# adamchang2000/DenseFusion

Hardware: AMD Instinct MI355X
Metric: poses/sec (node) YCB-Video 1000 pts + 2 refine iters (higher is better)
Workload: dtype f32

## Files before the change

densefusion_amd/_lib.py:

```python
from __future__ import annotations

import ctypes
import os

_HERE = os.path.dirname(os.path.abspath(__file__))
LIB_PATH = os.path.join(_HERE, "libdfusion_hip_dev.so" if os.environ.get("DF_DEV_LIB") else "libdfusion_hip.so")
_lib = None

_vp, _i, _i64, _f, _sz = ctypes.c_void_p, ctypes.c_int, ctypes.c_int64, ctypes.c_float, ctypes.c_size_t

class ConvDesc(ctypes.Structure):
    _fields_ = ([(n, ctypes.c_void_p) for n in ("in_", "wgt", "bias", "res", "prelu", "out")] +
                [(n, ctypes.c_int32) for n in ("B", "H", "W", "Cin", "in_ld", "in_coff", "OH", "OW", "Cout", "out_ld",
                                               "out_coff", "res_ld", "res_coff", "KH", "KW", "stride", "pad", "dil",
                                               "act")] +
                [("splitk_ws", ctypes.c_void_p), ("splitk_ws_bytes", ctypes.c_size_t)])


SIGNATURES = {
    "df_last_error": (ctypes.c_char_p, []),
    "df_version": (_i, []),
    "df_knn_device": (_i, [_vp, _i, _vp, _i, _i, _i, _vp, _vp]),
    "df_knn": (_i, [_vp, _vp, _vp, _i, _i, _i, _i, _i, _vp]),
    "knn_device": (None, [_vp, _i, _vp, _i, _i, _i, _vp, _vp, _vp]),
# ... 73 lines not shown
    "df_conv_route": (_i, [ctypes.POINTER(ConvDesc), _i, _vp, _vp, _vp, _i, _i, _i, _i, _vp]),
    "df_conv3x3_winograd_scratch_bytes": (ctypes.c_size_t, [ctypes.POINTER(ConvDesc)]),
    "df_conv3x3_winograd_nhwc": (_i, [ctypes.POINTER(ConvDesc), _vp, ctypes.c_size_t, _vp]),
    "df_wino_route": (_i, [_i, _i, _i, _i, _i]),
    "df_wino_tiles": (ctypes.c_long, [_i, _i, _i, _i, _i, ctypes.POINTER(_i), ctypes.POINTER(_i)]),
    "df_wino_axis_map": (_i, [_i, _i, _i, _i]),
    "df_trainer_create": (_vp, [_i, _i, _i]),
    "df_trainer_destroy": (None, [_vp]),
    "df_trainer_flat_numel": (_i64, [_vp]),
    "df_trainer_num_params": (_i, [_vp]),
    "df_trainer_param_info": (_i, [_vp, _i, ctypes.c_char_p, _i, ctypes.POINTER(_i64), ctypes.POINTER(_i)]),
    "df_trainer_pack_param": (_i, [_vp, ctypes.c_char_p, _vp, _vp, _vp]),
    "df_trainer_unpack_param": (_i, [_vp, ctypes.c_char_p, _vp, _vp, _vp]),
    "df_posenet_train_workspace_bytes": (_sz, [_vp, _i, _i, _i, _i]),
    "df_posenet_train_step": (_i, [_vp, _vp, _vp, _i64, _i, _i, _i] + [_vp] * 6 + [_i, _vp, _f, _i, ctypes.c_uint] + [_vp] * 9 + [_sz, _vp]),
    "df_posenet_train_multi_workspace_bytes": (_sz, [_vp, _i, _vp, _vp, _vp, _i]),
    "df_posenet_train_step_multi": (_i, [_vp, _vp, _vp, _i64, _i, _vp, _vp, _vp, _vp] + [_vp] * 5 + [_i, _vp, _f, _i, ctypes.c_uint] + [_vp] * 9 + [_sz, _vp]),
    "df_trainer_set_splitk": (_i, [_vp, _i]),
    "df_trainer_profile": (_i, [_vp, _i]),
    "df_trainer_profile_read": (_i, [_vp, ctypes.POINTER(ctypes.c_double), ctypes.POINTER(ctypes.c_double), ctypes.POINTER(_i)]),
    "df_refiner_train_workspace_bytes": (_sz, [_vp, _i, _i]),
    "df_refiner_train_step": (_i, [_vp, _vp, _vp, _i64, _i] + [_vp] * 5 + [_i, _vp] + [_vp] * 4 + [_sz, _vp]),
    "df_conv3x3_winograd_tile_scratch_bytes": (ctypes.c_size_t, [ctypes.POINTER(ConvDesc), _i]),
    "df_conv3x3_winograd_tile_nhwc": (_i, [ctypes.POINTER(ConvDesc), _i, _vp, ctypes.c_size_t, _vp]),
    "df_conv2d_dgrad_nhwc": (_i, [ctypes.POINTER(ConvDesc), _vp, _vp, _vp, _i, _vp]),
    "df_conv2d_wgrad_workspace_bytes": (ctypes.c_size_t, [ctypes.POINTER(ConvDesc)]),
    "df_conv2d_wgrad_nhwc": (_i, [ctypes.POINTER(ConvDesc), _vp, _vp, _vp, _vp, ctypes.c_size_t, _vp]),
    "df_net_debug_taps": (_i, [_vp, _i]),
    "df_net_debug_tap_read": (_i, [_vp, ctypes.c_char_p, _vp, _i64, ctypes.POINTER(_i64)]),
    "df_net_profile": (_i, [_vp, _i]),
    "df_net_profile_read": (_i, [_vp] + [ctypes.POINTER(ctypes.c_double)] * 4 + [ctypes.POINTER(_i)]),
    "df_net_profile_read_split": (_i, [_vp] + [ctypes.POINTER(ctypes.c_double)] * 3 + [ctypes.POINTER(_i)]),
    "df_gemm_route": (_i, [_i, _i, _i]),
    "df_segment_scratch_bytes": (_sz, [_i, _i, _i, _i]),
    "df_segment_input": (_i, [_vp, _vp, _i, _i, _i, _vp]),
    "df_segment_detect": (_i, [_vp, _vp, _i, _i, _i, _i, _i, _i, _i, _vp, _vp, _vp, _vp, _vp, _sz, _vp]),
    "df_seg_batch_scratch_bytes": (_sz, [_i, _i, _i, _i]),
    "df_seg_batch": (_i, [_vp, _vp, _i, _i, _i, _vp, _i, _i, _i, _vp, _i, _i, _vp, _i, _i, _i, _i, _i, _vp, _vp, _vp, _vp, _sz, _vp]),
    "df_seg_score_block_pixels": (_i, []),
    "df_seg_score": (_i, [_vp, _vp, _i, _i, _i, _i, _i, _vp, _vp, _vp, _vp]),
    "df_seg_masks": (_i, [_vp, _i, _i, _i, _vp, _vp, _i, _i, _i, _vp, _vp]),
    "df_mesh_closest_tile_triangles": (_i, []),
    "df_mesh_closest_scratch_bytes": (_sz, [_i]),
    "df_mesh_closest": (_i, [_vp, _i, _vp, _i, _vp, _i, _vp, _i, _vp, _vp, _vp, _vp, _sz, _vp]),
    "df_fp64_rate_probe": (_i, [_i, _i, _vp, _vp]),
}


def lib():
    global _lib
    if _lib is None:
        if not os.path.exists(LIB_PATH):
            raise RuntimeError(
                f"{LIB_PATH} not found: the HIP extension is not built. Run "
                "`python -c 'import __graft_entry__ as g; g.build()'` at the repo root (needs hipcc). "
                "densefusion_amd has no CPU fallback.")
        L = ctypes.CDLL(LIB_PATH)
        for name, (res, args) in SIGNATURES.items():
            fn = getattr(L, name)
            fn.restype, fn.argtypes = res, args
        _lib = L
    return _lib


def check(status: int, what: str = "") -> None:
    if status != 0:
# ... 38 lines not shown
```

densefusion_amd/csrc/conv_api.hip:

```cpp
#include <vector>

#include "igemm.h"
#include "wino.h"

using namespace df;

extern "C" int df_gemm_route(int n, int k, int epilogue) { return split_route(n, k, epilogue); }

static void desc_fields(const df_conv_desc *d, ConvParams &p) {
  p.in = d->in; p.wgt = d->wgt; p.bias = d->bias; p.res = d->res; p.prelu = d->prelu; p.out = d->out;
  p.B = d->B; p.H = d->H; p.W = d->W; p.Cin = d->Cin; p.in_ld = d->in_ld; p.in_coff = d->in_coff;
  p.OH = d->OH; p.OW = d->OW; p.Cout = d->Cout; p.out_ld = d->out_ld; p.out_coff = d->out_coff;
  p.res_ld = d->res_ld; p.res_coff = d->res_coff;
  p.KH = d->KH; p.KW = d->KW; p.stride = d->stride; p.pad = d->pad; p.dil = d->dil; p.act = d->act;
}

static int conv_desc_to_params(const df_conv_desc *d, ConvParams &p, const char *what) {
  if (!d) return set_error(DF_ERR_ARG, "%s: null descriptor", what);
  if (d->KH != d->KW) return set_error(DF_ERR_ARG, "%s: square kernels only", what);
  desc_fields(d, p);
  if (p.OH != conv_out(p.H, p.KH, p.stride, p.pad, p.dil) || p.OW != conv_out(p.W, p.KW, p.stride, p.pad, p.dil))
    return set_error(DF_ERR_ARG, "%s: OH/OW do not match the convolution geometry", what);
  return DF_OK;
}

static thread_local int t_last_splitk = 1;
extern "C" int df_conv_last_splitk(void) { return t_last_splitk; }

extern "C" int df_conv2d_nhwc(const df_conv_desc *d, df_stream_t stream) {
  ConvParams p;
  int rc = conv_desc_to_params(d, p, "conv2d_nhwc");
  if (rc != DF_OK) return rc;
  if (p.act == ACT_PRELU && !p.prelu) return set_error(DF_ERR_ARG, "conv2d_nhwc: PReLU needs a slope");
  p.splitk_ws = static_cast<float *>(d->splitk_ws); p.splitk_ws_bytes = d->splitk_ws ? d->splitk_ws_bytes : 0;
  ConvRoute taken;
  rc = launch_conv(p, to_stream(stream), &taken);
  t_last_splitk = taken.splitk;
  return rc;
}

// ... 191 lines not shown
```

densefusion_amd/csrc/igemm.h:

```cpp
#pragma once
#include "common.h"

namespace df {

enum Act { ACT_NONE = 0, ACT_RELU = 1, ACT_PRELU = 2 };

struct ConvParams {
  const float *in = nullptr;
  const float *wgt = nullptr;
  const float *bias = nullptr;
  const float *res = nullptr;
  const float *prelu = nullptr;
  float *out = nullptr;
  float *colsum = nullptr;
  int B = 1, H = 1, W = 1, Cin = 0, in_ld = 0, in_coff = 0;
  int OH = 1, OW = 1, Cout = 0, out_ld = 0, out_coff = 0;
  int res_ld = 0, res_coff = 0;
  int KH = 1, KW = 1, stride = 1, pad = 0, dil = 1;
  int up = 1;
  int act = ACT_NONE;
  int rows_per_group = 0, rows_valid = 0, bias_group_ld = 0;
  int zcount = 1;
  long z_in_coff = 0, z_wgt = 0, z_bias = 0, z_out_coff = 0;
  const void *wpl = nullptr;
// ... 13 lines not shown
  q.B = f.B; q.H = f.OH; q.W = f.OW; q.Cin = f.Cout; q.OH = f.H; q.OW = f.W; q.Cout = f.Cin;
  q.KH = f.KH; q.KW = f.KW; q.stride = 1; q.up = f.stride; q.dil = f.dil; q.pad = f.dil * (f.KH - 1) - f.pad;
  return q;
}

struct WgradSeg { int B, H, W, OH, OW; long in_row0, out_row0; };

enum ConvKernel { CONV_NONE = 0, CONV_V1 = 1, CONV_V2 = 2, CONV_V4 = 3, CONV_V4_COLSUM = 4, CONV_V4_MULTI = 5, CONV_BF16 = 6 };
struct ConvRoute {
  int kernel = CONV_NONE;
  int bm = 0, bn = 0;
  int loader = 0;
  int splitk = 1;
  int wgroup = 0;
  int nseg = 1;
};
int conv_route(const ConvParams &p, int nseg, const WgradSeg *segs, int first, ConvRoute &r);
int launch_conv(const ConvParams &p, hipStream_t st, ConvRoute *taken = nullptr);

constexpr int CONV_MAX_BUCKETS = 16;
int launch_conv_multi(const ConvParams &p, int nseg, const WgradSeg *segs, hipStream_t st);

size_t wgrad_workspace_bytes(const ConvParams &p);
int launch_wgrad(const ConvParams &p, float *dw, float *db, void *ws, size_t ws_bytes, hipStream_t st, int accumulate = 0);

constexpr int WGRAD_MAX_SEGS = 32;
size_t wgrad_multi_workspace_bytes(const ConvParams &p, int nseg, const WgradSeg *segs);
int launch_wgrad_multi(const ConvParams &p, int nseg, const WgradSeg *segs, float *dw, float *db, void *ws, size_t ws_bytes, hipStream_t st,
                       int accumulate = 0);

enum GemmEpi { GEMM_EPI_PLAIN = 0, GEMM_EPI_RESIDUAL = 1, GEMM_EPI_GROUPS = 2, GEMM_EPI_OTHER = 3 };
int gemm_epi_kind(const ConvParams &p);
int split_route(int N, int K, int epi);
void cut_weight_planes(const float *w, void *planes, long elems, long stride, hipStream_t st);
int try_split_gemm(const ConvParams &p, hipStream_t st, ConvRoute &r);

}
```

densefusion_amd/csrc/split_gemm.hip:

```cpp
#include "igemm.h"
#include <atomic>
#include <cstdint>
#ifdef DF_DEV
#include <map>
#include <mutex>
#include <tuple>
#endif

namespace df {
namespace {

typedef __bf16 bf16x8 __attribute__((ext_vector_type(8)));
typedef __bf16 bf16x2 __attribute__((ext_vector_type(2)));
typedef float f32x16 __attribute__((ext_vector_type(16)));
typedef float f32x2 __attribute__((ext_vector_type(2)));

constexpr int SBM = 128, SBN = 128, SBK = 32;
constexpr int PLANE_BYTES = 128 * 64;

__device__ __forceinline__ void cut3(float a0, float a1, unsigned &hi, unsigned &mid, unsigned &lo) {
  const bf16x2 h = __builtin_convertvector(f32x2{a0, a1}, bf16x2);
  hi = __builtin_bit_cast(unsigned, h);
  const float r0 = a0 - __builtin_bit_cast(float, hi << 16), r1 = a1 - __builtin_bit_cast(float, hi & 0xFFFF0000u);
  const bf16x2 m = __builtin_convertvector(f32x2{r0, r1}, bf16x2);
// ... 7 lines not shown
__device__ __forceinline__ void cut4(const float4 &x, uint4 &h, uint4 &m, uint4 &l) {
  if (H == 0) { cut3(x.x, x.y, h.x, m.x, l.x); cut3(x.z, x.w, h.y, m.y, l.y); }
  else { cut3(x.x, x.y, h.z, m.z, l.z); cut3(x.z, x.w, h.w, m.w, l.w); }
}
__device__ __forceinline__ void cut8(const float4 &x0, const float4 &x1, uint4 &h, uint4 &m, uint4 &l) { cut4<0>(x0, h, m, l); cut4<1>(x1, h, m, l); }

__host__ __device__ constexpr int pair_a(int q) { constexpr int t[6] = {2, 0, 1, 1, 0, 0}; return t[q]; }
__host__ __device__ constexpr int pair_b(int q) { constexpr int t[6] = {0, 2, 1, 0, 1, 0}; return t[q]; }
__device__ __forceinline__ f32x16 mfma_pair(const bf16x8 (&fa)[3], const bf16x8 (&fb)[3], int q, f32x16 c) {
  return __builtin_amdgcn_mfma_f32_32x32x16_bf16(fa[pair_a(q)], fb[pair_b(q)], c, 0, 0, 0);
}
constexpr bool pair_brings_new_planes(int q) {
  for (int r = 0; r < q; ++r)
    if (pair_a(r) == pair_a(q) || pair_b(r) == pair_b(q)) return false;
  return true;
}
static_assert(pair_brings_new_planes(0) && pair_brings_new_planes(1) && pair_brings_new_planes(2), "pairs 0..2 must reach all planes of A and of B");

__global__ void cut_planes_kernel(const float *__restrict__ w, __bf16 *__restrict__ planes, long elems, long stride) {
  const long i = (long)blockIdx.x * blockDim.x + threadIdx.x;
  if (i >= elems) return;
  unsigned h, m, l;
  cut3(w[i], 0.f, h, m, l);
  unsigned short *pl = reinterpret_cast<unsigned short *>(planes);
  pl[i] = (unsigned short)h; pl[stride + i] = (unsigned short)m; pl[2 * stride + i] = (unsigned short)l;
}

struct SplitArgs {
  const float *in; const __bf16 *wpl; const float *bias; const float *res; const float *prelu; float *out; float *colsum;
  long M, wplane;
  int N, K, in_ld, in_coff, out_ld, out_coff, res_ld, res_coff, act, rows_per_group, rows_valid, bias_group_ld;
  long z_in_coff, z_wgt, z_bias, z_out_coff;
  int tiles_m, tiles_n;
  long cs_rows;
};

__device__ __forceinline__ int piece(int row, int slot) { return row * 64 + ((slot ^ ((row >> 2) & 3)) << 4); }

struct SplitTile { int tm, tn, z; const float *in; const __bf16 *wpl; };
__device__ __forceinline__ bool split_tile(const SplitArgs &a, SplitTile &t) {
  const int xcd = blockIdx.x & 7, seq = blockIdx.x >> 3;
  t.tm = (seq / a.tiles_n) * 8 + xcd;
  t.tn = seq % a.tiles_n;
  t.z = blockIdx.z;
  t.in = a.in + t.z * a.z_in_coff + a.in_coff;
  t.wpl = a.wpl + t.z * a.z_wgt;
  return t.tm < a.tiles_m;
}

#define SPLIT_FETCH3(p0, p1, p2, g, k0)                                          \
  do {                                                                           \
    p0 = *reinterpret_cast<const uint4 *>((g) + (k0));                           \
    p1 = *reinterpret_cast<const uint4 *>((g) + a.wplane + (k0));                \
    p2 = *reinterpret_cast<const uint4 *>((g) + 2 * a.wplane + (k0));            \
  } while (0)
#define SPLIT_STORE3(base, stride, off, p0, p1, p2)                              \
  do {                                                                           \
    *reinterpret_cast<uint4 *>((base) + (off)) = p0;                             \
    *reinterpret_cast<uint4 *>((base) + (stride) + (off)) = p1;                  \
    *reinterpret_cast<uint4 *>((base) + 2 * (stride) + (off)) = p2;              \
  } while (0)
#define SPLIT_FRAG_OFFSETS(b0)                                                   \
  int offa[2][2], offb[2][2];                                                    \
  _Pragma("unroll") for (int ks = 0; ks < 2; ++ks)                               \
  _Pragma("unroll") for (int t = 0; t < 2; ++t) {                                \
    offa[ks][t] = piece(wr * 64 + t * 32 + fr, ks * 2 + fh);                     \
    offb[ks][t] = (b0) + piece(wc * 64 + t * 32 + fr, ks * 2 + fh);              \
  }
#define SPLIT_READ_FRAGS(base, apl, bpl)                                                                  \
  bf16x8 fa[2][3], fb[2][3];                                                                              \
  _Pragma("unroll") for (int t = 0; t < 2; ++t)                                                           \
  _Pragma("unroll") for (int p = 0; p < 3; ++p) {                                                         \
    fa[t][p] = *reinterpret_cast<const bf16x8 *>((base) + p * (apl) + offa[ks][t]);                       \
    fb[t][p] = *reinterpret_cast<const bf16x8 *>((base) + p * (bpl) + offb[ks][t]);                       \
  }
#define SPLIT_STAGE_ROLES(half)                                                  \
  const int srow0 = tid >> 2, srow1 = srow0 + (half), sslot = tid & 3;           \
  const int soff0 = piece(srow0, sslot), soff1 = piece(srow1, sslot);            \
  long r0 = row0 + srow0, r1 = row0 + srow1;                                     \
  r0 = r0 < a.M ? r0 : a.M - 1;                                                  \
// ... 59 lines not shown
  const EpiRules ru = epi_rules(a, z, row0, wrow);
  float *out = a.out + z * a.z_out_coff + a.out_coff;
#pragma unroll
  for (int j = 0; j < 2; ++j) {
    const int n = nb + j * 32 + fr;
    const float b1 = ru.bias ? ru.bias[n] : 0.f;
    float csum = 0.f;
#pragma unroll
    for (int i = 0; i < 2; ++i) {
      const int tb = wrow + i * 32 + 4 * fh;
      const long mb = row0 + tb;
      float r[16];
      if (a.res) {
#pragma unroll
        for (int e = 0; e < 16; ++e) {
          long m = mb + (e & 3) + 8 * (e >> 2);
          m = m < a.M ? m : a.M - 1;
          r[e] = a.res[m * a.res_ld + a.res_coff + n];
        }
      }
#pragma unroll
      for (int e = 0; e < 16; ++e) {
        const int tr = tb + (e & 3) + 8 * (e >> 2);
        const long m = row0 + tr;
        const float v = epi_finish(acc[i][j][e], &b1, a.res ? &r[e] : nullptr, a.act, ru.slope);
        if (a.out && m < a.M) out[m * a.out_ld + n] = v;
        csum += tr < ru.limit ? v : 0.f;
      }
    }
    epi_colsum(a, ru, z, n, fh, csum);
  }
}

__device__ __forceinline__ void split_epilogue_rows(const SplitArgs &a, const f32x16 (&acc)[2][2], int z, long row0, int wrow, int nb, int lane, float *blk) {
  const int fr = lane & 31, fh = lane >> 5;
  const EpiRules ru = epi_rules(a, z, row0, wrow);
#pragma unroll
  for (int j = 0; j < 2; ++j) {
    const int n = nb + j * 32 + fr;
    const float b1 = ru.bias ? ru.bias[n] : 0.f;
    float csum = 0.f;
#pragma unroll
    for (int i = 0; i < 2; ++i)
#pragma unroll
      for (int e = 0; e < 16; ++e) {
        const int br = i * 32 + 4 * fh + (e & 3) + 8 * (e >> 2);
        const float v = a.res ? epi_finish(acc[i][j][e], &b1, nullptr, ACT_NONE, 0.f) : epi_finish(acc[i][j][e], &b1, nullptr, a.act, ru.slope);
        blk[br * 64 + j * 32 + fr] = v;
        csum += wrow + br < ru.limit ? v : 0.f;
      }
    epi_colsum(a, ru, z, n, fh, csum);
  }
  if (!a.out) return;
  __builtin_amdgcn_fence(__ATOMIC_RELEASE, "wavefront");
  __builtin_amdgcn_wave_barrier();
  __builtin_amdgcn_fence(__ATOMIC_ACQUIRE, "wavefront");
  float *out = a.out + z * a.z_out_coff + a.out_coff;
  const int c4 = (lane & 15) * 4;
#pragma unroll 4
  for (int it = 0; it < 16; ++it) {
    const int br = it * 4 + (lane >> 4);
    const long m = row0 + wrow + br;
    float4 v = *reinterpret_cast<const float4 *>(blk + br * 64 + c4);
    if (m < a.M) {
      if (a.res) {
        const float4 r = *reinterpret_cast<const float4 *>(a.res + m * a.res_ld + a.res_coff + nb + c4);
        epi_finish(reinterpret_cast<float (&)[4]>(v), nullptr, &r.x, a.act, ru.slope);
      }
      *reinterpret_cast<float4 *>(out + m * a.out_ld + nb + c4) = v;
    }
  }
  __builtin_amdgcn_fence(__ATOMIC_RELEASE, "wavefront");
  __builtin_amdgcn_wave_barrier();
}

__global__ __launch_bounds__(256, 2) void gemm_split_bf16_kernel(const SplitArgs a) {
  __shared__ __attribute__((aligned(16))) unsigned char lds[6 * PLANE_BYTES];
  const int tid = threadIdx.x, lane = tid & 63, wave = tid >> 6;
  SplitTile wg;
  if (!split_tile(a, wg)) return;
  const long row0 = (long)wg.tm * SBM;
  const int n0 = wg.tn * SBN;

  SPLIT_STAGE_ROLES(64);
  const __bf16 *bg1 = wg.wpl + (long)(n0 + srow1) * a.K + sslot * 8;
// ... 93 lines not shown
    __builtin_amdgcn_sched_group_barrier(0x020, 7, 0);                           \
    __builtin_amdgcn_sched_group_barrier(0x100, 12, 0);                          \
    _Pragma("unroll") for (int g = 0; g < 48; ++g) {                             \
      __builtin_amdgcn_sched_group_barrier(0x008, 1, 0);                         \
      __builtin_amdgcn_sched_group_barrier(0x002, 2, 0);                         \
      if (g >= 8 && g < 32 && (g & 1) == 0) __builtin_amdgcn_sched_group_barrier(0x100, 1, 0); \
      if (g % 5 == 4) __builtin_amdgcn_sched_group_barrier(0x200, 1, 0);         \
    }                                                                            \
    __syncthreads();                                                             \
  } while (0)

  unsigned char *const st0 = lds2, *const st1 = lds2 + V2_STAGE;
  const int nk = a.K / SBK;
  const int klast = a.K - SBK;
  V2_FETCH(x, 0);
  V2_FETCH(y, SBK < klast ? SBK : klast);
  V2_STAGE_TO(x, st0);
  __syncthreads();
  int kt = 0;
  for (; kt + 1 < nk; kt += 2) {
    const int k2 = (kt + 2) * SBK, k3 = (kt + 3) * SBK;
    V2_BODY(x, y, k2 < klast ? k2 : klast, st0, st1);
    V2_BODY(y, x, k3 < klast ? k3 : klast, st1, st0);
  }
  if (nk & 1) { V2_COMPUTE(st0); }
  split_epilogue(a, acc, wg.z, row0, wr * 64, n0 + wc * 64, fr, fh);
}

constexpr int V3_PL = 256 * 32, V3_STAGE = 6 * V3_PL;
constexpr int V3_LDS = 8 * 64 * 64 * 4;

__device__ __forceinline__ int piece16(int row, int half) { return row * 32 + ((half ^ ((row >> 3) & 1)) << 4); }

__global__ __launch_bounds__(512, 1) void gemm_split_bf16_v3_kernel(const SplitArgs a) {
  extern __shared__ __attribute__((aligned(16))) unsigned char lds3[];
  const int tid = threadIdx.x, lane = tid & 63, wave = tid >> 6;
  SplitTile wg;
  if (!split_tile(a, wg)) return;
  const long row0 = (long)wg.tm * 256;
  const int n0 = wg.tn * 256;

  const int srow = tid >> 1, shalf = tid & 1;
  const int soff = piece16(srow, shalf);
  long r = row0 + srow;
  r = r < a.M ? r : a.M - 1;
  const float *ag = wg.in + r * a.in_ld + shalf * 8;
  const __bf16 *bg = wg.wpl + (long)(n0 + srow) * a.K + shalf * 8;
  float4 xa0, xa1, ya0, ya1;
  uint4 b0, b1, b2;
#define V3_FETCH_A(S, k0)                                                        \
  do {                                                                           \
    S##a0 = *reinterpret_cast<const float4 *>(ag + (k0));                        \
    S##a1 = *reinterpret_cast<const float4 *>(ag + (k0) + 4);                    \
  } while (0)
#define V3_FETCH_B(k0) SPLIT_FETCH3(b0, b1, b2, bg, k0)
#define V3_PIN(v) asm volatile("" : "+v"(v.x), "+v"(v.y), "+v"(v.z), "+v"(v.w))
#define V3_CUT0(S) do { V3_PIN(S##a0); cut4<0>(S##a0, ch, cm, cl); } while (0)
#define V3_CUT1(S) do { V3_PIN(S##a1); cut4<1>(S##a1, ch, cm, cl); } while (0)
#define V3_WRITE_A(base) SPLIT_STORE3(base, V3_PL, soff, ch, cm, cl)
#define V3_WRITE_B(base) SPLIT_STORE3((base) + 3 * V3_PL, V3_PL, soff, b0, b1, b2)

  const int wr = wave >> 2, wc = wave & 3, fr = lane & 31, fh = lane >> 5;
  f32x16 acc[2][2][2] = {};
  const int offa = piece16(wr * 128 + fr, fh), offb = 3 * V3_PL + piece16(wc * 64 + fr, fh);
#define V3_READ(base, q)                                                                                  \
  do {                                                                                                    \
    _Pragma("unroll") for (int t = 0; t < 4; ++t)                                                         \
      fa[t][pair_a(q)] = *reinterpret_cast<const bf16x8 *>((base) + pair_a(q) * V3_PL + offa + t * 1024); \
    _Pragma("unroll") for (int t = 0; t < 2; ++t)                                                         \
      fb[t][pair_b(q)] = *reinterpret_cast<const bf16x8 *>((base) + pair_b(q) * V3_PL + offb + t * 1024); \
  } while (0)
#define V3_MFMA(q)                                                                                        \
  do {                                                                                                    \
    _Pragma("unroll") for (int i = 0; i < 4; ++i)                                                         \
    _Pragma("unroll") for (int j = 0; j < 2; ++j) acc[i >> 1][i & 1][j] = mfma_pair(fa[i], fb[j], q, acc[i >> 1][i & 1][j]); \
  } while (0)
#define V3_WEAVE(n, mask, cnt)                                                   \
  do {                                                                           \
    _Pragma("unroll") for (int g = 0; g < (n); ++g) {                            \
      __builtin_amdgcn_sched_group_barrier(0x008, 1, 0);                         \
      __builtin_amdgcn_sched_group_barrier(mask, cnt, 0);                        \
    }                                                                            \
    __builtin_amdgcn_sched_barrier(0);                                           \
  } while (0)
#define V3_BODY(FS, SS, ka, kb, cur, nxt)                                        \
  do {                                                                           \
    bf16x8 fa[4][3], fb[2][3];                                                   \
    uint4 ch, cm, cl;                                                            \
    V3_FETCH_B(kb);                                                              \
    V3_FETCH_A(FS, ka);                                                          \
    V3_READ(cur, 0);                                                             \
    __builtin_amdgcn_sched_barrier(0);                                           \
    V3_READ(cur, 1);                                                             \
    V3_MFMA(0);                                                                  \
    V3_WEAVE(6, 0x100, 1);                                                       \
    V3_READ(cur, 2);                                                             \
    V3_MFMA(1);                                                                  \
    V3_WEAVE(6, 0x100, 1);                                                       \
    V3_CUT0(SS);                                                                 \
    V3_MFMA(2);                                                                  \
    V3_WEAVE(8, 0x002, 3);                                                       \
    V3_CUT1(SS);                                                                 \
    V3_MFMA(3);                                                                  \
    V3_WEAVE(8, 0x002, 3);                                                       \
    V3_WRITE_A(nxt);                                                             \
    V3_MFMA(4);                                                                  \
    V3_WEAVE(3, 0x200, 1);                                                       \
    V3_WRITE_B(nxt);                                                             \
    V3_MFMA(5);                                                                  \
    V3_WEAVE(3, 0x200, 1);                                                       \
    __syncthreads();                                                             \
  } while (0)

  unsigned char *const st0 = lds3, *const st1 = lds3 + V3_STAGE;
  const int nk = a.K / 16;
  const int klast = a.K - 16;
  V3_FETCH_B(0);
  V3_FETCH_A(x, 0);
  V3_FETCH_A(y, 16);
  {
    uint4 ch, cm, cl;
    V3_CUT0(x);
    V3_CUT1(x);
    V3_WRITE_A(st0);
    V3_WRITE_B(st0);
  }
  __syncthreads();
  for (int s = 0; s < nk; s += 2) {
    const int k1 = (s + 1) * 16, k2 = (s + 2) * 16, k3 = (s + 3) * 16;
    V3_BODY(x, y, k2 < klast ? k2 : klast, k1, st0, st1);
    V3_BODY(y, x, k3 < klast ? k3 : klast, k2 < klast ? k2 : klast, st1, st0);
  }
  float *const blk = reinterpret_cast<float *>(lds3) + wave * (64 * 64);
  split_epilogue_rows(a, acc[0], wg.z, row0, wr * 128, n0 + wc * 64, lane, blk);
  split_epilogue_rows(a, acc[1], wg.z, row0, wr * 128 + 64, n0 + wc * 64, lane, blk);
}

#ifdef DF_DEV
std::mutex g_mu;
std::map<std::tuple<int, hipStream_t>, std::pair<__bf16 *, long>> g_scratch;

const __bf16 *scratch_planes(const float *w, long elems, hipStream_t st) {
  int dev = 0;
  (void)hipGetDevice(&dev);
  std::lock_guard<std::mutex> g(g_mu);
  auto &sc = g_scratch[std::make_tuple(dev, st)];
  if (sc.second < elems) {
    if (sc.first) (void)hipFree(sc.first);
    sc = {nullptr, 0};
    if (hipMalloc(reinterpret_cast<void **>(&sc.first), (size_t)elems * 3 * sizeof(__bf16)) != hipSuccess) return nullptr;
    sc.second = elems;
  }
  cut_weight_planes(w, sc.first, elems, elems, st);
  return sc.first;
}
#endif

enum SplitForm { FORM_128x128 = 0, FORM_256x128 = 1, FORM_256x256 = 2 };
struct FormDesc { const char *name; void (*kernel)(SplitArgs); int bm, bn, threads, lds; bool raise; };
const FormDesc FORMS[3] = {{"128x128", gemm_split_bf16_kernel, SBM, SBN, 256, 0, false},
                           {"256x128", gemm_split_bf16_v2_kernel, 256, SBN, 512, 2 * V2_STAGE, true},
                           {"256x256", gemm_split_bf16_v3_kernel, 256, 256, 512, V3_LDS, true}};

struct SplitPlan {
  bool examined = false;
  int form = FORM_128x128;
  int threads = 0, lds = 0;
  dim3 grid;
  SplitArgs a{};
};

int plan_split(const ConvParams &p, int compute_units, int variant, bool all, SplitPlan &pl) {
  pl = SplitPlan{};
  if (p.splitk_ws || (!p.wpl && !all)) return 0;
  pl.examined = true;
  const long M = (long)p.B * p.OH * p.OW;
  const int K = p.Cin;
  SplitArgs &a = pl.a;
  a.in = p.in; a.wpl = reinterpret_cast<const __bf16 *>(p.wpl); a.bias = p.bias; a.res = p.res; a.prelu = p.prelu; a.out = p.out; a.colsum = p.colsum;
  a.M = M; a.wplane = p.wpl_stride; a.N = p.Cout; a.K = K; a.in_ld = p.in_ld; a.in_coff = p.in_coff; a.out_ld = p.out_ld; a.out_coff = p.out_coff;
  a.res_ld = p.res_ld; a.res_coff = p.res_coff; a.act = p.act; a.rows_per_group = p.rows_per_group; a.rows_valid = p.rows_valid; a.bias_group_ld = p.bias_group_ld;
  a.z_in_coff = p.z_in_coff; a.z_wgt = p.z_wgt; a.z_bias = p.z_bias; a.z_out_coff = p.z_out_coff;
  a.cs_rows = colsum_partial_rows(M);
  const bool ok = p.KH == 1 && p.KW == 1 && p.stride == 1 && p.pad == 0 && p.up == 1 && p.H == p.OH && p.W == p.OW && (p.out || p.colsum) &&
                  p.Cout % SBN == 0 && K % SBK == 0 && K >= SBK && M >= 1 && gemm_epi_kind(p) != GEMM_EPI_OTHER &&
                  (p.rows_per_group == 0 ? p.bias_group_ld == 0 : p.rows_per_group % SBM == 0) && (p.z_wgt % 8) == 0;
  if (!ok || !(all || split_route(p.Cout, K, gemm_epi_kind(p)))) {
    if (p.wpl && !all) return set_error(DF_ERR_ARG, "split gemm: routed launch M=%ld N=%d K=%d outside the kernels' cover", M, p.Cout, K);
    return 0;
  }
  const bool v2 = variant >= 2 && K >= 384 && (p.rows_per_group == 0 || p.rows_per_group % 256 == 0);
  const long tiles3 = ((M + 255) / 256) * (p.Cout / 256) * p.zcount;
  const bool rows16 = (!p.out || (reinterpret_cast<uintptr_t>(p.out) % 16 == 0 && p.out_ld % 4 == 0 && p.out_coff % 4 == 0 && p.z_out_coff % 4 == 0)) &&
                      (!p.res || (reinterpret_cast<uintptr_t>(p.res) % 16 == 0 && p.res_ld % 4 == 0 && p.res_coff % 4 == 0));
  const bool v3 = v2 && variant >= 3 && p.Cout % 256 == 0 && rows16 && tiles3 >= compute_units;
  pl.form = v3 ? FORM_256x256 : v2 ? FORM_256x128 : FORM_128x128;
  const FormDesc &f = FORMS[pl.form];
  a.tiles_m = (int)((M + f.bm - 1) / f.bm);
  a.tiles_n = p.Cout / f.bn;
  pl.grid = dim3((unsigned)(((a.tiles_m + 7) / 8) * 8 * a.tiles_n), 1, p.zcount);
  pl.threads = f.threads;
  pl.lds = f.lds;
  return 1;
}

}

int split_route(int N, int K, int epi) {
  if (N <= 0 || N % SBN != 0 || K % SBK != 0 || K < 384) return 0;
  return epi == GEMM_EPI_PLAIN || epi == GEMM_EPI_RESIDUAL || epi == GEMM_EPI_GROUPS;
}

int gemm_epi_kind(const ConvParams &p) {
  const bool groups = p.rows_per_group > 0 || p.bias_group_ld > 0 || p.colsum;
  if (p.res) return groups ? GEMM_EPI_OTHER : GEMM_EPI_RESIDUAL;
  return groups ? GEMM_EPI_GROUPS : GEMM_EPI_PLAIN;
}

void cut_weight_planes(const float *w, void *planes, long elems, long stride, hipStream_t st) {
  hipLaunchKernelGGL(cut_planes_kernel, dim3((unsigned)((elems + 255) / 256)), dim3(256), 0, st, w, reinterpret_cast<__bf16 *>(planes), elems, stride);
}

static int compute_units() {
  static std::atomic<int> cus[64];
  int dev = 0;
  (void)hipGetDevice(&dev);
  if (dev < 0 || dev >= 64) return 256;
  int n = cus[dev].load(std::memory_order_relaxed);
  if (n == 0) {
    if (hipDeviceGetAttribute(&n, hipDeviceAttributeMultiprocessorCount, dev) != hipSuccess || n <= 0) n = 256;
    cus[dev].store(n, std::memory_order_relaxed);
  }
  return n;
}

int try_split_gemm(const ConvParams &p, hipStream_t st, ConvRoute &r) {
  static const bool off = dev_getenv("DF_GEMM_SPLIT_OFF") != nullptr;
  static const bool all = dev_getenv("DF_GEMM_SPLIT_BF16") != nullptr;
  static const bool verbose = dev_getenv("DF_GEMM_SPLIT_VERBOSE") != nullptr;
  static const int variant = dev_getenv("DF_GEMM_SPLIT_V") ? atoi(dev_getenv("DF_GEMM_SPLIT_V")) : 3;
  if (off) return 0;
  SplitPlan pl;
  const int rc = plan_split(p, compute_units(), variant, all, pl);
  if (verbose && pl.examined) fprintf(stderr, "[df-split] M=%ld N=%d K=%d z%d -> %s\n", pl.a.M, p.Cout, p.Cin, p.zcount, rc == 1 ? "bf16 x 6" : "fp32");
  if (rc != 1) return rc;
#ifdef DF_DEV
  if (!pl.a.wpl) {
    pl.a.wplane = (long)(p.zcount - 1) * p.z_wgt + (long)p.Cout * p.Cin;
    pl.a.wpl = scratch_planes(p.wgt, pl.a.wplane, st);
    if (!pl.a.wpl) return set_error(DF_ERR_LAUNCH, "split gemm: hipMalloc of the weight-plane scratch failed");
  }
#endif
  const FormDesc &f = FORMS[pl.form];
  if (verbose) fprintf(stderr, "[df-split]   form %s\n", f.name);
  if (f.raise) {
    const int e = raise_lds_limit(reinterpret_cast<const void *>(f.kernel), pl.lds);
    if (e != DF_OK) return e;
  }
  hipLaunchKernelGGL(f.kernel, pl.grid, dim3(pl.threads), pl.lds, st, pl.a);
  r = ConvRoute{};
  r.kernel = CONV_BF16;
  r.bm = f.bm;
  r.bn = f.bn;
  return 1;
}

}
```

include/dfusion.h:

```cpp
#ifndef DFUSION_H_
#define DFUSION_H_

#include <stddef.h>
#include <stdint.h>

#ifdef __cplusplus
extern "C" {
#endif

typedef void *df_stream_t;

#define DF_OK 0
#define DF_ERR_ARG (-1)
#define DF_ERR_LAUNCH (-2)
#define DF_ERR_WORKSPACE (-3)
#define DF_ERR_STATE (-4)

const char *df_last_error(void);
int df_version(void);

#define DF_KNN_MAX_K 32
int df_knn_device(const float *ref_dev, int ref_nb, const float *query_dev, int query_nb, int dim, int k,
                  int64_t *ind_dev, df_stream_t stream);

// ... 215 lines not shown
int df_trainer_num_params(const df_trainer *t);
int df_trainer_param_info(const df_trainer *t, int i, char *key_out, int key_cap, int64_t *shape4, int *ndim);
int df_trainer_pack_param(const df_trainer *t, const char *key, const float *src, float *flat, df_stream_t stream);
int df_trainer_unpack_param(const df_trainer *t, const char *key, const float *flat, float *dst, df_stream_t stream);
size_t df_posenet_train_workspace_bytes(const df_trainer *t, int B, int H, int W, int M);
int df_posenet_train_step(df_trainer *t, const float *flat_param, float *flat_grad, int64_t param_version, int B, int H, int W,
                          const float *img, const float *cloud, const int64_t *choose, const int64_t *obj, const float *target,
                          const float *model_points, int M, const int *symmetric_host, float w, int dropout, unsigned seed,
                          float *loss_out, float *dis_out, float *new_points, float *new_target, float *out_r, float *out_t,
                          float *out_c, float *emb, void *ws, size_t ws_bytes, df_stream_t stream);
size_t df_posenet_train_multi_workspace_bytes(const df_trainer *t, int nb, const int *B, const int *H, const int *W, int M);
int df_posenet_train_step_multi(df_trainer *t, const float *flat_param, float *flat_grad, int64_t param_version, int nb, const int *B,
                                const int *H, const int *W, const float *const *img, const float *cloud, const int64_t *choose,
                                const int64_t *obj, const float *target, const float *model_points, int M, const int *symmetric_host,
                                float w, int dropout, unsigned seed, float *loss_out, float *dis_out, float *new_points,
                                float *new_target, float *out_r, float *out_t, float *out_c, float *emb, void *ws, size_t ws_bytes,
                                df_stream_t stream);
int df_trainer_set_splitk(df_trainer *t, int enable);
int df_trainer_profile(df_trainer *t, int enable);
int df_trainer_profile_read(df_trainer *t, double *ms3, double *flops3, int *launches3);
size_t df_refiner_train_workspace_bytes(const df_trainer *t, int B, int M);
int df_refiner_train_step(df_trainer *t, const float *flat_param, float *flat_grad, int64_t param_version, int B, const float *points,
                          const float *emb, const int64_t *obj, const float *target, const float *model_points, int M,
                          const int *symmetric_host, float *dis_out, float *new_points, float *new_target, void *ws, size_t ws_bytes,
                          df_stream_t stream);

int df_net_profile(df_net *net, int enable);
int df_net_profile_read(df_net *net, double *gemm_ms, double *gemm_flops, double *gemm_useful_flops, double *gemm_bytes,
                        int *launches);
int df_net_profile_read_split(df_net *net, double *gemm_ms, double *gemm_flops, double *gemm_useful_flops, int *launches);

int df_gemm_route(int n, int k, int epilogue);

int df_net_debug_taps(df_net *net, int enable);
int df_net_debug_tap_read(df_net *net, const char *name, float *dst, int64_t cap, int64_t *shape4);

#ifdef __cplusplus
}
#endif
#endif
```

Baseline: 10480.

## Make v3 split bf16 GEMM persistent with tile walk and prefetch overlap

Result: faster. 10700 (median of 6 runs) (+2.1%).

```diff
diff --git a/densefusion_amd/_lib.py b/densefusion_amd/_lib.py
--- a/densefusion_amd/_lib.py
+++ b/densefusion_amd/_lib.py
@@ -129,6 +129,8 @@
     "df_net_profile_read": (_i, [_vp] + [ctypes.POINTER(ctypes.c_double)] * 4 + [ctypes.POINTER(_i)]),
     "df_net_profile_read_split": (_i, [_vp] + [ctypes.POINTER(ctypes.c_double)] * 3 + [ctypes.POINTER(_i)]),
     "df_gemm_route": (_i, [_i, _i, _i]),
+    "df_split_walk": (_i, [_i, _i, _i, _i, ctypes.POINTER(_i), ctypes.POINTER(_i), ctypes.POINTER(_i), _i]),
+    "df_gemm_rows": (_i, [_vp] * 6 + [_i64, _i, _i, _i, _i, _i, _i, _i, _vp]),
     "df_segment_scratch_bytes": (_sz, [_i, _i, _i, _i]),
     "df_segment_input": (_i, [_vp, _vp, _i, _i, _i, _vp]),
     "df_segment_detect": (_i, [_vp, _vp, _i, _i, _i, _i, _i, _i, _i, _vp, _vp, _vp, _vp, _vp, _sz, _vp]),
diff --git a/densefusion_amd/csrc/conv_api.hip b/densefusion_amd/csrc/conv_api.hip
--- a/densefusion_amd/csrc/conv_api.hip
+++ b/densefusion_amd/csrc/conv_api.hip
@@ -6,6 +6,32 @@
 using namespace df;
 
 extern "C" int df_gemm_route(int n, int k, int epilogue) { return split_route(n, k, epilogue); }
+
+extern "C" int df_split_walk(int tiles_m, int tiles_n, int zcount, int workgroups, int *grid, int *tiles_total, int *trips, int cap) {
+  if (tiles_m <= 0 || tiles_n <= 0 || zcount <= 0 || (long)((tiles_m + 7) / 8) * 8 * tiles_n * zcount >= (1L << 30))
+    return set_error(DF_ERR_ARG, "split_walk: need positive tile counts with fewer than 2^30 positions");
+  const SplitWalk w = split_walk(tiles_m, tiles_n, zcount, workgroups);
+  if (grid) *grid = w.grid;
+  if (tiles_total) *tiles_total = w.tiles_total;
+  for (int b = 0; trips && b < w.grid && b < cap; ++b) trips[b] = split_walk_trips(w, b);
+  return DF_OK;
+}
+
+extern "C" int df_gemm_rows(const float *in, const float *wgt, const float *bias, const float *res, float *out, float *colsum, int64_t M, int N,
+                            int K, int zcount, int act, int rows_per_group, int rows_valid, int bias_group_ld, df_stream_t stream) {
+  if (!in || !wgt || (!out && !colsum)) return set_error(DF_ERR_ARG, "gemm_rows: null pointer");
+  if (M <= 0 || M >= (1L << 31) || N <= 0 || K <= 0 || zcount <= 0) return set_error(DF_ERR_ARG, "gemm_rows: bad shape");
+  if (act != ACT_NONE && act != ACT_RELU) return set_error(DF_ERR_ARG, "gemm_rows: activation must be none or ReLU");
+  if (rows_per_group < 0 || (rows_per_group == 0 ? rows_valid != 0 || bias_group_ld != 0 : M % rows_per_group != 0 || rows_valid <= 0 || rows_valid > rows_per_group))
+    return set_error(DF_ERR_ARG, "gemm_rows: row groups must divide M, with 1 .. rows_per_group real rows each");
+  if (zcount > 1 && (res || bias_group_ld > 0)) return set_error(DF_ERR_ARG, "gemm_rows: a z batch takes neither a residual nor per-group bias");
+  ConvParams p;
+  p.in = in; p.wgt = wgt; p.bias = bias; p.res = res; p.out = out; p.colsum = colsum;
+  p.B = (int)M; p.Cin = K; p.in_ld = K; p.Cout = N; p.out_ld = N; p.res_ld = N; p.act = act;
+  p.rows_per_group = rows_per_group; p.rows_valid = rows_valid; p.bias_group_ld = bias_group_ld;
+  p.zcount = zcount; p.z_in_coff = M * K; p.z_wgt = (long)N * K; p.z_bias = bias ? N : 0; p.z_out_coff = M * N;
+  return launch_conv(p, to_stream(stream));
+}
 
 static void desc_fields(const df_conv_desc *d, ConvParams &p) {
   p.in = d->in; p.wgt = d->wgt; p.bias = d->bias; p.res = d->res; p.prelu = d->prelu; p.out = d->out;
diff --git a/densefusion_amd/csrc/igemm.h b/densefusion_amd/csrc/igemm.h
--- a/densefusion_amd/csrc/igemm.h
+++ b/densefusion_amd/csrc/igemm.h
@@ -69,6 +69,9 @@
 enum GemmEpi { GEMM_EPI_PLAIN = 0, GEMM_EPI_RESIDUAL = 1, GEMM_EPI_GROUPS = 2, GEMM_EPI_OTHER = 3 };
 int gemm_epi_kind(const ConvParams &p);
 int split_route(int N, int K, int epi);
+struct SplitWalk { int grid, tiles_total; };
+SplitWalk split_walk(int tiles_m, int tiles_n, int zcount, int workgroups);
+int split_walk_trips(const SplitWalk &w, int b);
 void cut_weight_planes(const float *w, void *planes, long elems, long stride, hipStream_t st);
 int try_split_gemm(const ConvParams &p, hipStream_t st, ConvRoute &r);
 
diff --git a/densefusion_amd/csrc/split_gemm.hip b/densefusion_amd/csrc/split_gemm.hip
--- a/densefusion_amd/csrc/split_gemm.hip
+++ b/densefusion_amd/csrc/split_gemm.hip
@@ -63,20 +63,27 @@
   int N, K, in_ld, in_coff, out_ld, out_coff, res_ld, res_coff, act, rows_per_group, rows_valid, bias_group_ld;
   long z_in_coff, z_wgt, z_bias, z_out_coff;
   int tiles_m, tiles_n;
+  int tiles_total;
   long cs_rows;
 };
 
 __device__ __forceinline__ int piece(int row, int slot) { return row * 64 + ((slot ^ ((row >> 2) & 3)) << 4); }
 
 struct SplitTile { int tm, tn, z; const float *in; const __bf16 *wpl; };
-__device__ __forceinline__ bool split_tile(const SplitArgs &a, SplitTile &t) {
-  const int xcd = blockIdx.x & 7, seq = blockIdx.x >> 3;
+__device__ __forceinline__ bool split_tile_at(const SplitArgs &a, int xcd, int seq, int z, SplitTile &t) {
   t.tm = (seq / a.tiles_n) * 8 + xcd;
   t.tn = seq % a.tiles_n;
-  t.z = blockIdx.z;
+  t.z = z;
   t.in = a.in + t.z * a.z_in_coff + a.in_coff;
   t.wpl = a.wpl + t.z * a.z_wgt;
   return t.tm < a.tiles_m;
+}
+__device__ __forceinline__ bool split_tile(const SplitArgs &a, SplitTile &t) { return split_tile_at(a, blockIdx.x & 7, blockIdx.x >> 3, blockIdx.z, t); }
+__device__ __forceinline__ bool split_walk_next(const SplitArgs &a, int &seq, SplitTile &t) {
+  const int seq_z = ((a.tiles_m + 7) >> 3) * a.tiles_n;
+  for (; seq < (a.tiles_total >> 3); seq += (int)(gridDim.x >> 3))
+    if (split_tile_at(a, blockIdx.x & 7, seq % seq_z, seq / seq_z, t)) return true;
+  return false;
 }
 
 #define SPLIT_FETCH3(p0, p1, p2, g, k0)                                          \
@@ -202,9 +209,8 @@
   }
 }
 
-__device__ __forceinline__ void split_epilogue_rows(const SplitArgs &a, const f32x16 (&acc)[2][2], int z, long row0, int wrow, int nb, int lane, float *blk) {
-  const int fr = lane & 31, fh = lane >> 5;
-  const EpiRules ru = epi_rules(a, z, row0, wrow);
+template <int ACT>
+__device__ __forceinline__ void split_block_to_lds(const SplitArgs &a, const f32x16 (&acc)[2][2], const EpiRules &ru, int z, int wrow, int nb, int fr, int fh, float *blk) {
 #pragma unroll
   for (int j = 0; j < 2; ++j) {
     const int n = nb + j * 32 + fr;
@@ -215,12 +221,20 @@
 #pragma unroll
       for (int e = 0; e < 16; ++e) {
         const int br = i * 32 + 4 * fh + (e & 3) + 8 * (e >> 2);
-        const float v = a.res ? epi_finish(acc[i][j][e], &b1, nullptr, ACT_NONE, 0.f) : epi_finish(acc[i][j][e], &b1, nullptr, a.act, ru.slope);
+        const float v = epi_finish(acc[i][j][e], &b1, nullptr, ACT, ru.slope);
         blk[br * 64 + j * 32 + fr] = v;
         csum += wrow + br < ru.limit ? v : 0.f;
       }
     epi_colsum(a, ru, z, n, fh, csum);
   }
+}
+__device__ __forceinline__ void split_epilogue_rows(const SplitArgs &a, const f32x16 (&acc)[2][2], int z, long row0, int wrow, int nb, int lane, float *blk) {
+  const int fr = lane & 31, fh = lane >> 5;
+  const EpiRules ru = epi_rules(a, z, row0, wrow);
+  const int act = a.res ? ACT_NONE : a.act;
+  if (act == ACT_RELU) split_block_to_lds<ACT_RELU>(a, acc, ru, z, wrow, nb, fr, fh, blk);
+  else if (act == ACT_PRELU) split_block_to_lds<ACT_PRELU>(a, acc, ru, z, wrow, nb, fr, fh, blk);
+  else split_block_to_lds<ACT_NONE>(a, acc, ru, z, wrow, nb, fr, fh, blk);
   if (!a.out) return;
   __builtin_amdgcn_fence(__ATOMIC_RELEASE, "wavefront");
   __builtin_amdgcn_wave_barrier();
@@ -380,20 +394,32 @@
 
 __device__ __forceinline__ int piece16(int row, int half) { return row * 32 + ((half ^ ((row >> 3) & 1)) << 4); }
 
+#ifndef DF_STRACE
+#define DF_STRACE_ENTRY()
+#define DF_STRACE(i, s) ((void)(s))
+#endif
+
 __global__ __launch_bounds__(512, 1) void gemm_split_bf16_v3_kernel(const SplitArgs a) {
   extern __shared__ __attribute__((aligned(16))) unsigned char lds3[];
   const int tid = threadIdx.x, lane = tid & 63, wave = tid >> 6;
+  DF_STRACE_ENTRY();
   SplitTile wg;
-  if (!split_tile(a, wg)) return;
-  const long row0 = (long)wg.tm * 256;
-  const int n0 = wg.tn * 256;
+  int seq = blockIdx.x >> 3;
+  if (!split_walk_next(a, seq, wg)) return;
 
   const int srow = tid >> 1, shalf = tid & 1;
   const int soff = piece16(srow, shalf);
-  long r = row0 + srow;
-  r = r < a.M ? r : a.M - 1;
-  const float *ag = wg.in + r * a.in_ld + shalf * 8;
-  const __bf16 *bg = wg.wpl + (long)(n0 + srow) * a.K + shalf * 8;
+  const float *ag;
+  const __bf16 *bg;
+#define V3_TILE_ROLES()                                                          \
+  do {                                                                           \
+    int t = tid;                                                                 \
+    asm volatile("" : "+v"(t));                                                  \
+    long r = (long)wg.tm * 256 + (t >> 1);                                       \
+    r = r < a.M ? r : a.M - 1;                                                   \
+    ag = wg.in + r * a.in_ld + (t & 1) * 8;                                      \
+    bg = wg.wpl + (long)(wg.tn * 256 + (t >> 1)) * a.K + (t & 1) * 8;            \
+  } while (0)
   float4 xa0, xa1, ya0, ya1;
   uint4 b0, b1, b2;
 #define V3_FETCH_A(S, k0)                                                        \
@@ -409,7 +435,6 @@
 #define V3_WRITE_B(base) SPLIT_STORE3((base) + 3 * V3_PL, V3_PL, soff, b0, b1, b2)
 
   const int wr = wave >> 2, wc = wave & 3, fr = lane & 31, fh = lane >> 5;
-  f32x16 acc[2][2][2] = {};
   const int offa = piece16(wr * 128 + fr, fh), offb = 3 * V3_PL + piece16(wc * 64 + fr, fh);
 #define V3_READ(base, q)                                                                                  \
   do {                                                                                                    \
@@ -463,25 +488,56 @@
   unsigned char *const st0 = lds3, *const st1 = lds3 + V3_STAGE;
   const int nk = a.K / 16;
   const int klast = a.K - 16;
-  V3_FETCH_B(0);
-  V3_FETCH_A(x, 0);
-  V3_FETCH_A(y, 16);
-  {
-    uint4 ch, cm, cl;
-    V3_CUT0(x);
-    V3_CUT1(x);
-    V3_WRITE_A(st0);
-    V3_WRITE_B(st0);
-  }
-  __syncthreads();
-  for (int s = 0; s < nk; s += 2) {
-    const int k1 = (s + 1) * 16, k2 = (s + 2) * 16, k3 = (s + 3) * 16;
-    V3_BODY(x, y, k2 < klast ? k2 : klast, k1, st0, st1);
-    V3_BODY(y, x, k3 < klast ? k3 : klast, k2 < klast ? k2 : klast, st1, st0);
-  }
-  float *const blk = reinterpret_cast<float *>(lds3) + wave * (64 * 64);
-  split_epilogue_rows(a, acc[0], wg.z, row0, wr * 128, n0 + wc * 64, lane, blk);
-  split_epilogue_rows(a, acc[1], wg.z, row0, wr * 128 + 64, n0 + wc * 64, lane, blk);
+#define V3_FIRST_FETCHES()                                                       \
+  do {                                                                           \
+    V3_TILE_ROLES();                                                             \
+    V3_FETCH_B(0);                                                               \
+    V3_FETCH_A(x, 0);                                                            \
+    V3_FETCH_A(y, 16);                                                           \
+  } while (0)
+  V3_FIRST_FETCHES();
+  DF_STRACE(0, seq);
+  DF_STRACE(1, seq);
+  for (;;) {
+    const long row0 = (long)wg.tm * 256;
+    const int n0 = wg.tn * 256, z = wg.z, seq0 = seq;
+    f32x16 acc[2][2][2] = {};
+    {
+      uint4 ch, cm, cl;
+      V3_CUT0(x);
+      V3_CUT1(x);
+      V3_WRITE_A(st0);
+      V3_WRITE_B(st0);
+    }
+    __syncthreads();
+    DF_STRACE(2, seq0);
+    for (int s = 0; s < nk; s += 2) {
+      const int k1 = (s + 1) * 16, k2 = (s + 2) * 16, k3 = (s + 3) * 16;
+      V3_BODY(x, y, k2 < klast ? k2 : klast, k1, st0, st1);
+      V3_BODY(y, x, k3 < klast ? k3 : klast, k2 < klast ? k2 : klast, st1, st0);
+    }
+    DF_STRACE(3, seq0);
+    seq += (int)(gridDim.x >> 3);
+    const bool more = split_walk_next(a, seq, wg);
+    if (more) {
+      V3_FIRST_FETCHES();
+      DF_STRACE(1, seq);
+    }
+    __builtin_amdgcn_sched_barrier(0);
+    int et = tid;
+    asm volatile("" : "+v"(et));
+    const int elane = et & 63, ewr = et >> 8, ewc = (et >> 6) & 3;
+    float *const blk = reinterpret_cast<float *>(lds3) + (et >> 6) * (64 * 64);
+    split_epilogue_rows(a, acc[0], z, row0, ewr * 128, n0 + ewc * 64, elane, blk);
+    DF_STRACE(4, seq0);
+    split_epilogue_rows(a, acc[1], z, row0, ewr * 128 + 64, n0 + ewc * 64, elane, blk);
+    DF_STRACE(5, seq0);
+    if (!more) {
+      DF_STRACE(6, seq0);
+      break;
+    }
+    __syncthreads();
+  }
 }
 
 #ifdef DF_DEV
@@ -518,7 +574,7 @@
   SplitArgs a{};
 };
 
-int plan_split(const ConvParams &p, int compute_units, int variant, bool all, SplitPlan &pl) {
+int plan_split(const ConvParams &p, int compute_units, int variant, bool all, int workgroups, SplitPlan &pl) {
   pl = SplitPlan{};
   if (p.splitk_ws || (!p.wpl && !all)) return 0;
   pl.examined = true;
@@ -541,12 +597,17 @@
   const long tiles3 = ((M + 255) / 256) * (p.Cout / 256) * p.zcount;
   const bool rows16 = (!p.out || (reinterpret_cast<uintptr_t>(p.out) % 16 == 0 && p.out_ld % 4 == 0 && p.out_coff % 4 == 0 && p.z_out_coff % 4 == 0)) &&
                       (!p.res || (reinterpret_cast<uintptr_t>(p.res) % 16 == 0 && p.res_ld % 4 == 0 && p.res_coff % 4 == 0));
-  const bool v3 = v2 && variant >= 3 && p.Cout % 256 == 0 && rows16 && tiles3 >= compute_units;
+  const bool v3 = v2 && variant >= 3 && p.Cout % 256 == 0 && rows16 && tiles3 >= compute_units && tiles3 < (1L << 27);
   pl.form = v3 ? FORM_256x256 : v2 ? FORM_256x128 : FORM_128x128;
   const FormDesc &f = FORMS[pl.form];
   a.tiles_m = (int)((M + f.bm - 1) / f.bm);
   a.tiles_n = p.Cout / f.bn;
   pl.grid = dim3((unsigned)(((a.tiles_m + 7) / 8) * 8 * a.tiles_n), 1, p.zcount);
+  if (v3) {
+    const SplitWalk w = split_walk(a.tiles_m, a.tiles_n, p.zcount, workgroups < 0 ? compute_units : workgroups);
+    a.tiles_total = w.tiles_total;
+    pl.grid = dim3((unsigned)w.grid, 1, 1);
+  }
   pl.threads = f.threads;
   pl.lds = f.lds;
   return 1;
@@ -557,6 +618,18 @@
 int split_route(int N, int K, int epi) {
   if (N <= 0 || N % SBN != 0 || K % SBK != 0 || K < 384) return 0;
   return epi == GEMM_EPI_PLAIN || epi == GEMM_EPI_RESIDUAL || epi == GEMM_EPI_GROUPS;
+}
+
+SplitWalk split_walk(int tiles_m, int tiles_n, int zcount, int workgroups) {
+  SplitWalk w;
+  w.tiles_total = ((tiles_m + 7) / 8) * 8 * tiles_n * zcount;
+  w.grid = workgroups <= 0 || workgroups >= w.tiles_total ? w.tiles_total : workgroups < 8 ? 8 : workgroups / 8 * 8;
+  return w;
+}
+
+int split_walk_trips(const SplitWalk &w, int b) {
+  const int seqs = w.tiles_total / 8, step = w.grid / 8, first = b / 8;
+  return first < seqs ? (seqs - first + step - 1) / step : 0;
 }
 
 int gemm_epi_kind(const ConvParams &p) {
@@ -587,9 +660,10 @@
   static const bool all = dev_getenv("DF_GEMM_SPLIT_BF16") != nullptr;
   static const bool verbose = dev_getenv("DF_GEMM_SPLIT_VERBOSE") != nullptr;
   static const int variant = dev_getenv("DF_GEMM_SPLIT_V") ? atoi(dev_getenv("DF_GEMM_SPLIT_V")) : 3;
+  static const int workgroups = dev_getenv("DF_GEMM_SPLIT_WGS") ? atoi(dev_getenv("DF_GEMM_SPLIT_WGS")) : -1;
   if (off) return 0;
   SplitPlan pl;
-  const int rc = plan_split(p, compute_units(), variant, all, pl);
+  const int rc = plan_split(p, compute_units(), variant, all, workgroups, pl);
   if (verbose && pl.examined) fprintf(stderr, "[df-split] M=%ld N=%d K=%d z%d -> %s\n", pl.a.M, p.Cout, p.Cin, p.zcount, rc == 1 ? "bf16 x 6" : "fp32");
   if (rc != 1) return rc;
 #ifdef DF_DEV
@@ -600,7 +674,7 @@
   }
 #endif
   const FormDesc &f = FORMS[pl.form];
-  if (verbose) fprintf(stderr, "[df-split]   form %s\n", f.name);
+  if (verbose) fprintf(stderr, "[df-split]   form %s\n[df-split]   workgroups %u\n", f.name, pl.grid.x * pl.grid.z);
   if (f.raise) {
     const int e = raise_lds_limit(reinterpret_cast<const void *>(f.kernel), pl.lds);
     if (e != DF_OK) return e;
diff --git a/include/dfusion.h b/include/dfusion.h
--- a/include/dfusion.h
+++ b/include/dfusion.h
@@ -271,6 +271,11 @@
 
 int df_gemm_route(int n, int k, int epilogue);
 
+int df_split_walk(int tiles_m, int tiles_n, int zcount, int workgroups, int *grid, int *tiles_total, int *trips, int cap);
+
+int df_gemm_rows(const float *in, const float *wgt, const float *bias, const float *res, float *out, float *colsum, int64_t M, int N,
+                 int K, int zcount, int act, int rows_per_group, int rows_valid, int bias_group_ld, df_stream_t stream);
+
 int df_net_debug_taps(df_net *net, int enable);
 int df_net_debug_tap_read(df_net *net, const char *name, float *dst, int64_t cap, int64_t *shape4);
 
```
